# davidlougheed/strkit

Measured on AMD Instinct MI355X. Metric: reads/sec realigned, higher is better.
Workload: dtype int32; 1 GPU; cfg2 shape (1000 loci x 30 HiFi reads, motif 3-6 bp, flank 70), 10000 loci x 30 reads per step and GPU, 8 distinct resident batches in rotation; exact scores (banded first pass with exactness certificate, exact fall-back); distinct_batches=8, parallelism=loci-sharded x1, calls_in_flight=2

## Files before the change

### strkit_amd/csrc/strk_dp_band.h

```cpp
#pragma once

namespace strk {

struct BandLayout {
    int wd, pad, maxdb, maxcol, off_sel, off_cp, cp_bytes, ct_bytes, cp_tail, off_ct, off_b0, group_bytes, sel_len;
    static constexpr int OFF_COMB = 0, OFF_MISC = OFF_COMB + kTableMax * 4, OFF_LMAX = OFF_MISC + 16;
    static constexpr int kBandHiPad = kBandRowSlack + 32;
    __host__ __device__ constexpr BandLayout(int c)
        : wd(128 << c), pad((128 << c) + (8 << c) + 8), maxdb(band_max_db(c)), maxcol(band_max_col(c)),
          off_sel(OFF_LMAX + (band_class_lmax(c) ? kTableMax * 4 : 0)),
          off_cp(off_sel + ((band_max_db(c) + 2 * ((128 << c) + (8 << c) + 8) + kBandHiPad + 15) & ~15)),
          cp_bytes(band_class_fly(c) ? 512 : ((band_max_db(c) + kBandRowSlack + 2 * (8 << c) + 4 + 15) & ~15)),
          ct_bytes((kBandMaxFlank + 2 * (8 << c) + 4 + 15) & ~15),
          cp_tail(c == 0 ? cp_bytes - ct_bytes : cp_bytes),
          off_ct(off_cp + cp_tail),
          off_b0(off_ct + ct_bytes),
          group_bytes(off_b0 + ((band_max_col(c) * 2 + 15) & ~15)),
          sel_len((band_max_db(c) + 2 * ((128 << c) + (8 << c) + 8) + kBandHiPad) & ~3) {}
};
static_assert(band_class_layout(4) == 0 && band_class_layout(7) == 3 && band_class_wd(5) <= band_class_wd(1) && band_class_G(6) == band_class_G(2),
              "a 12-diagonal class uses the LDS layout of the 16-diagonal class with its lane count: pads sized for the wider band cover it");
__host__ __device__ constexpr int band_wave_lds(int c) { return (64 / (8 << c)) * BandLayout(c).group_bytes; }
__host__ __device__ constexpr int max_band_wave_lds(int c) {
    return c < 0 ? 0 : (band_wave_lds(c) > max_band_wave_lds(c - 1) ? band_wave_lds(c) : max_band_wave_lds(c - 1));
}
constexpr int kBandWaveLds = max_band_wave_lds(3);
constexpr int kBandNeg16 = -20000;
constexpr int kBandTblClass0 = 18;
constexpr int kBandSelFront = 5, kBandSelBack = 6;
constexpr int kBandTblBytes = 256;
__host__ __device__ constexpr int band_class_symbol(int c) {
    return c == 0 ? 0 : (c == 1 ? 1 : (c == 2 ? 3 : (c == 3 ? 2 : (c == 4 ? 15 : (c == 7 ? 14 : -1)))));
}
constexpr unsigned kBandLetterLo = 0x47544341u, kBandLetterHi = 0x4E000058u;
typedef const __attribute__((address_space(3))) uint8_t* lds_cu8;

struct BandCtx {
    int lig;
    bool first, last;
    int notFirst, notLast;
    const uint8_t* tbl;
    const uint8_t* selb;
    int pad, maxidx, ndb;
    const uint8_t* flL;
    const uint8_t* motifL;
    int nfl, m;
    int flyP;
};

__device__ __forceinline__ int wave_min_over_groups(int v) {
    int m = __builtin_amdgcn_readlane(v, 0);
#pragma unroll
    for (int l = 8; l < 64; l += 8) m = min(m, __builtin_amdgcn_readlane(v, l));
    return m;
}
template <int G>
__device__ __forceinline__ int from_left0(int v, int notFirst) {
    const int x = __builtin_amdgcn_update_dpp(0, v, G <= 16 ? kDppRowShr1 : kDppWaveShr1, 0xf, 0xf, true);
    return (G == 16 || G == 64) ? x : (x & notFirst);
}
template <int G>
__device__ __forceinline__ int from_right0(int v, int notLast) {
    const int x = __builtin_amdgcn_update_dpp(0, v, G <= 16 ? kDppRowShl1 : kDppWaveShl1, 0xf, 0xf, true);
    return (G == 16 || G == 64) ? x : (x & notLast);
}

template <int G, int D, bool BWD, bool FLY, bool LMAX>
__device__ __forceinline__ void band_pass(const BandCtx& x, const uint8_t* rowsym, int nrows, int dlo_, bool topFree,
                                          bool leftFree, int nEff, int fork0, int m, int cmin, int ncol, int* comb,
                                          short* b0col, int* lmaxA) {
    static_assert(D % 4 == 0 && D >= 8 && D <= 16, "a lane keeps 8, 12 or 16 diagonals");
    constexpr int g = kGap, NQ = D / 4;
    const int ncols = x.ndb;
    const int d0 = dlo_ + x.lig * D;
    auto g0 = [&](int j) -> int { return topFree ? g * min(max(j, 0), ncols) : 0; };
    auto col_addr = [&](int j) -> int {
        return BWD ? x.pad + ncols - j : x.pad + j - 1;
    };
    int Ha[D], Hb[D];
    int Hsave[BWD ? D : 1];
    unsigned sel[NQ];
#pragma unroll
    for (int k = 0; k < (BWD ? D : 1); ++k) Hsave[k] = 0;
#pragma unroll
    for (int k = 0; k < D; ++k) Ha[k] = g0(-x.lig + d0 + k);
    const int jb0 = 1 - x.lig + d0;
    {
#pragma unroll
        for (int q = 0; q < NQ; ++q) {
            unsigned v = 0;
#pragma unroll
            for (int b = 0; b < 4; ++b) v |= (unsigned)x.selb[col_addr(jb0 + 4 * q + b)] << (8 * b);
            sel[q] = v;
        }
    }
    const int T = (wave_max_over_groups(nrows > 0 ? nrows + G - 1 : 0) + 1) & ~1;
    const int dhi_ = dlo_ + D * G - 1;
    int houtL = Ha[D - 1];
    int forkT = (!BWD && nEff > 0) ? fork0 - 1 + x.lig : 0x7fffffff;
    if (BWD && nrows > 0) forkT = nrows - 1 + x.lig;
    int forkIdx = 0;
    int lastmax = kNegInf;
    lds_cu8 psym = FLY ? (lds_cu8)(x.flL + 256 - x.nfl - x.lig) : (lds_cu8)(rowsym + (G - 1) - x.lig);
    lds_cu8 const flyEnd = (lds_cu8)x.motifL + x.flyP;
    lds_cu8 const tbl = (lds_cu8)x.tbl;
    auto row_word = [&](unsigned sym8) -> uint2 {
        const unsigned long long v = *reinterpret_cast<const __attribute__((address_space(3))) unsigned long long*>(tbl + sym8);
        return make_uint2((unsigned)v, (unsigned)(v >> 32));
    };
    uint2 wordE, wordO;
    wordE = row_word(psym[0]);
    wordO = row_word(psym[1]);
    lds_cu8 pnb = (lds_cu8)(x.selb + col_addr(jb0 + D)) - (BWD ? 1 : 0);
#define STRK_BAND_STEP(SRC, DST, TT, ODD, EDGE, FORK)                                              \
    {                                                                                              \
        if (FORK) { STRK_BAND_FORK(SRC, (TT) - 1) }                                                \
        const uint2 word = (ODD) ? wordO : wordE;                                                  \
        unsigned sym2 = (unsigned)psym[2 + (ODD)];                         \
        unsigned nb = pnb[BWD ? 1 - (ODD) : (ODD)];                                                \
        int leftEdge, keepU = 0;                                                                   \
        if (EDGE) {                                                                                \
              \
            const int keepL = ((TT) + dlo_ <= 0 && leftFree) ? g * ((TT) + 1) : 0;                  \
            leftEdge = from_left<G>(keepL, houtL, x.first);                                        \
              \
            const int rl = (TT) - G + 2;                                                           \
            keepU = rl <= 1 ? g0(rl + dhi_) : 0;                                                   \
        } else {                                                                                   \
            leftEdge = from_left0<G>(houtL, x.notFirst);                                           \
        }                                                                                          \
        unsigned wq[NQ];                                                                           \
        _Pragma("unroll") for (int q = 0; q < NQ; ++q) wq[q] = __builtin_amdgcn_perm(word.y, word.x, sel[q]); \
        DST[0] = max(max(SRC[1], leftEdge), SRC[0] + (int)(wq[0] & 0xffu));                        \
        const int upEdge = (EDGE) ? from_right<G>(keepU, DST[0], x.last) : from_right0<G>(DST[0], x.notLast); \
        _Pragma("unroll") for (int k = 1; k < D - 1; ++k)                                          \
            DST[k] = max(max(SRC[k + 1], DST[k - 1]), SRC[k] + (int)((wq[k / 4] >> (8 * (k % 4))) & 0xffu)); \
        DST[D - 1] = max(max(upEdge, DST[D - 2]), SRC[D - 1] + (int)(wq[NQ - 1] >> 24));           \
        houtL = DST[D - 1];                                                                        \
                          \
        asm volatile("" : "+v"(nb), "+v"(sym2));                                                   \
        if (LMAX && !BWD) {                                                                        \
            lastmax = max(lastmax + g, houtL);       \
                                                \
            if ((EDGE) && (TT) == G - 2) lastmax = kNegInf;                                        \
        }                                                                                          \
        _Pragma("unroll") for (int q = 0; q + 1 < NQ; ++q) sel[q] = __builtin_amdgcn_alignbyte(sel[q + 1], sel[q], 1); \
        sel[NQ - 1] = __builtin_amdgcn_alignbyte(nb, sel[NQ - 1], 1);                              \
        if (ODD) wordO = row_word(sym2); else wordE = row_word(sym2);                              \
    }
#define STRK_BAND_FORK(V, TT)                                                                      \
                                                                     \
    if ((!BWD || __builtin_amdgcn_ballot_w64((TT) == forkT) != 0) && (TT) == forkT) {              \
        const int jb = jb0 + (TT);                        \
        if (BWD) {                                                                                 \
                           \
            _Pragma("unroll") for (int k = 0; k < D; ++k)                                          \
                asm volatile("v_mov_b32 %0, %1" : "+v"(Hsave[k]) : "v"(V[k]));                         \
            forkT = 0x7fffffff;                                                                    \
        } else {                                                                                   \
            const short* bc = b0col + (jb - cmin);                                                 \
            int acc = kNegInf;                                                                     \
            _Pragma("unroll") for (int k = 0; k < D; k += 2)                                       \
                acc = max(max(acc, V[k] + (int)bc[k]), V[k + 1] + (int)bc[k + 1]);                 \
            atomicMax(&comb[forkIdx], acc);                                                        \
            if (LMAX && x.last) lmaxA[forkIdx] = lastmax - g * ((TT) + 1 - x.lig);    \
            ++forkIdx;                                                                             \
            forkT = forkIdx < nEff ? forkT + m : 0x7fffffff;                                       \
        }                                                                                          \
    }
    const bool hasL = nrows > 0 && leftFree && dlo_ <= 0;
    const int tTop = (G - 1) & ~1;
    const int tL0 = wave_min_over_groups(hasL ? -dlo_ : 0x3fffffff) & ~1;
    const int tL1 = wave_max_over_groups(hasL ? -dlo_ : -1);
    const int tF = min(T, wave_min_over_groups(BWD ? (nrows > 0 ? nrows - 1 : 0x3fffffff) : (nEff > 0 ? fork0 - 1 : 0x3fffffff)) & ~1);
    auto advance = [&]() {
        psym += 2;
        if (FLY) {
            int past = (int)(flyEnd - psym - 1) >> 31;
            asm volatile("" : "+v"(past));
            psym -= x.flyP & past;
        }
        asm volatile("" : "+v"(psym));
        pnb += BWD ? -2 : 2;
        asm volatile("" : "+v"(pnb));
    };
    int t = 0;
    while (t < T) {
        int ts = T;
        if (tTop >= t) ts = min(ts, tTop);
        if (tL1 >= t) ts = min(ts, max(tL0, t));
        for (const int tn = min(ts, tF); t < tn; t += 2) {
            STRK_BAND_STEP(Ha, Hb, t, 0, false, false)
            STRK_BAND_STEP(Hb, Ha, t + 1, 1, false, false)
            advance();
        }
        for (; t < ts; t += 2) {
            STRK_BAND_STEP(Ha, Hb, t, 0, false, true)
            STRK_BAND_STEP(Hb, Ha, t + 1, 1, false, true)
            advance();
        }
        for (; t < T && (t == tTop || (t >= tL0 && t <= tL1)); t += 2) {
            STRK_BAND_STEP(Ha, Hb, t, 0, true, true)
            STRK_BAND_STEP(Hb, Ha, t + 1, 1, true, true)
            advance();
        }
    }
    STRK_BAND_FORK(Ha, T - 1)
    if (BWD && nrows > 0) {
        const int jb = jb0 + nrows - 1 + x.lig;
#pragma unroll
        for (int k = 0; k < D; ++k) {
            const int jp = jb + k, idx = ncols - jp - cmin;
            if (jp >= 0 && jp <= ncols && idx >= 0 && idx < ncol) b0col[idx] = (short)Hsave[k];
        }
    }
#undef STRK_BAND_STEP
#undef STRK_BAND_FORK
}

template <int BC, class NA, class NB, class NC>
__device__ __forceinline__ void band_wave(const KArgs& a, bool act, int4 q0, int4 q1, int4 q2, uint8_t* Lw, const uint8_t* s_enc,
                                          const uint8_t* s_tbl, NA& nextA, NB& nextB, NC& nextC) {
    constexpr int g = kGap, G = band_class_G(BC), D = band_class_D(BC);
    constexpr bool FLY = band_class_fly(BC);
    constexpr bool LMAX = band_class_lmax(BC);
    constexpr BandLayout lay(band_class_layout(BC));
    const int lane = threadIdx.x & 63;
    int lig_ = lane & (G - 1);
    asm volatile("" : "+v"(lig_));
    const int lig = lig_;
    const int grp = lane / G;
    const bool first = lig == 0, last = lig == G - 1;
    uint8_t* const Lg = Lw + grp * lay.group_bytes;
    int* const comb = reinterpret_cast<int*>(Lg + BandLayout::OFF_COMB);
    int* const misc = reinterpret_cast<int*>(Lg + BandLayout::OFF_MISC);
    int* const lmaxA = reinterpret_cast<int*>(Lg + BandLayout::OFF_LMAX);
    uint8_t* const selb = Lg + lay.off_sel;
    uint8_t* const cp = Lg + lay.off_cp;
    uint8_t* const ct = Lg + lay.off_ct;
    short* const b0col = reinterpret_cast<short*>(Lg + lay.off_b0);
    uint8_t* const motifL = FLY ? cp + 256 : Lg + lay.off_b0;
    constexpr bool TAIL = lay.cp_tail < lay.cp_bytes;
    constexpr int kRowTail = lay.cp_tail - (G - 1);
    static_assert(2 * kBandMaxFlank + kGap * (kBandMaxFlank + band_max_db(1)) < 32767 + kBandNeg16, "b0col: 16-bit columns, kBandNeg16 as -inf");

    int r = 0, nfl = 1, ntr = 0, nfr = 1, m = 1, lo = 0, n = 0;
    long long soff = 0;
    const uint8_t* motif = a.motifs;
    if (act) {
        r = q0.x; nfl = q0.z; ntr = q0.w;
        nfr = q1.x; m = q1.y; lo = q1.z; n = q1.w;
        soff = (long long)(((unsigned long long)(unsigned)q2.y << 32) | (unsigned)q2.x);
        motif += q2.z;
    }
    const int ndb = nfl + ntr + nfr;
    const BandGeo geo = band_geometry_of_class(BC, nfl, ntr, m, lo, max(n, 1), a.band_tune);
    const int rowsP = act ? nfl + (lo + n - 1) * m : 0;
    const int rowsT = act ? nfr : 0;
    const bool dbBeg = a.end_flags & 1, dbEnd = a.end_flags & 2, cBeg = a.end_flags & 4, cEnd = a.end_flags & 8;

    if (first) { misc[0] = 0; misc[1] = act ? q2.z : 0; }
    wave_lds_sync();
    {
        constexpr unsigned kFront = 0x01010101u * kBandSelFront, kBack = 0x01010101u * kBandSelBack;
        constexpr int ND = lay.sel_len / 4, PD = lay.pad / 4;
        constexpr int kBehind = (lay.wd + kBandRowSlack + G + 28 + 3) / 4;
        static_assert(lay.pad % 4 == 0, "the window starts on a dword of the selector array");
        unsigned other = 0;
        const uint8_t* seq = a.seqs + soff;
        unsigned* const selw = reinterpret_cast<unsigned*>(selb);
        const int nd = act ? (ndb + 3) >> 2 : 0;
        for (int d = lig; d < PD; d += G) selw[d] = kFront;
        for (int d = PD + nd + lig; d < min(ND, PD + nd + kBehind); d += G) selw[d] = kBack;
        for (int d0 = lig; d0 < nd; d0 += 8 * G) {
            unsigned w[8];
#pragma unroll
            for (int u = 0; u < 8; ++u) {
                const int d = d0 + u * G;
                unsigned v = 0;
                if (4 * d + 3 < ndb) {
                    __builtin_memcpy(&v, seq + 4 * d, 4);
                } else {
#pragma unroll
                    for (int b = 0; b < 3; ++b)
                        if (4 * d + b < ndb) v |= (unsigned)seq[4 * d + b] << (8 * b);
                }
                w[u] = v;
            }
#pragma unroll
            for (int u = 0; u < 8; ++u) {
                const int d = d0 + u * G;
                unsigned out = (w[u] >> 1) & 0x07070707u;
                unsigned bad = (w[u] & 0xDFDFDFDFu) ^ __builtin_amdgcn_perm(kBandLetterHi, kBandLetterLo, out);
                if (4 * d + 3 >= ndb) {
                    const unsigned vm = 4 * d >= ndb ? 0u : (0xffffffffu >> (8 * (4 * d + 4 - ndb)));
                    out = (out & vm) | (kBack & ~vm);
                    bad &= vm;
                }
                other |= bad;
                if (d < nd) selw[PD + d] = out;
            }
        }
        nextA();
        if (other) misc[0] = 1;
        for (int k = lig; k < m; k += G) motifL[k] = act ? s_enc[motif[k]] : (uint8_t)kNullSym;
    }
    wave_lds_sync();
    const bool fallback = act && misc[0] != 0;
    for (int e = lig; e < kTableMax; e += G) { comb[e] = kNegInf; if (LMAX) lmaxA[e] = kNegInf; }
    {
        if (FLY) {
            for (int k = lig; k < 256; k += G) {
                const int row = k - (256 - nfl);
                cp[k] = (uint8_t)(8 * (row >= 0 ? kBandTblClass0 + selb[lay.pad + row] : kNullSym));
            }
            wave_lds_sync();
            for (int k = lig; k < m; k += G) motifL[k] = (uint8_t)(8 * motifL[k]);
            wave_lds_sync();
            for (int k = m + lig; k < 256; k += G) motifL[k] = motifL[k % m];
        } else {
            const int lenP = wave_max_over_groups(rowsP) + 2 * (G - 1) + 4;
            for (int idx = lig; idx < G - 1; idx += G) cp[idx] = (uint8_t)(8 * kNullSym);
            uint8_t* const cpr = cp + (G - 1);
            for (int row = lig; row < min(min(nfl, rowsP), kRowTail); row += G) cpr[row] = (uint8_t)(8 * (kBandTblClass0 + selb[lay.pad + row]));
            {
                const int gstep = G % m;
                int ph = lig % m;
                for (int row = nfl + lig; row < min(rowsP, kRowTail); row += G) {
                    cpr[row] = (uint8_t)(8 * motifL[ph]);
                    ph += gstep;
                    if (ph >= m) ph -= m;
                }
            }
            for (int row = rowsP + lig; row < min(lenP - (G - 1), kRowTail); row += G) cpr[row] = (uint8_t)(8 * kNullSym);
        }
        const int lenT = wave_max_over_groups(rowsT) + 2 * (G - 1) + 4;
        for (int idx = lig; idx < lenT; idx += G) {
            const int row = idx - (G - 1);
            int sym = kNullSym;
            if (row >= 0 && row < rowsT) sym = kBandTblClass0 + selb[lay.pad + ndb - 1 - row];
            ct[idx] = (uint8_t)(8 * sym);
        }
    }
    wave_lds_sync();
    {
        constexpr unsigned kNeg2 = ((unsigned)(unsigned short)(short)kBandNeg16) * 0x00010001u;
        const int nc2 = min(lay.maxcol, wave_max_over_groups(act ? geo.ncol : 0) + 1) >> 1;
        unsigned* const b2 = reinterpret_cast<unsigned*>(b0col);
        for (int k = lig; k <= nc2; k += G) if (2 * k < lay.maxcol) b2[k] = kNeg2;
    }
    wave_lds_sync();
    nextB();

    if (FLY) {
        const int rmax = wave_max_over_groups(rowsP);
        if (rmax >= 11264) __builtin_amdgcn_s_setprio(3);
        else if (rmax >= 8192) __builtin_amdgcn_s_setprio(2);
        else if (rmax >= 5120) __builtin_amdgcn_s_setprio(1);
    }
    BandCtx x;
    x.lig = lig; x.first = first; x.last = last; x.notFirst = first ? 0 : -1; x.notLast = last ? 0 : -1; x.selb = selb;
    asm volatile("" : "+v"(x.notFirst), "+v"(x.notLast));
    x.pad = lay.pad; x.maxidx = lay.sel_len - 1; x.ndb = ndb;
    x.flL = cp; x.motifL = motifL; x.nfl = nfl; x.m = m;
    x.flyP = FLY ? ((256 - 4) / m) * m : 0;
    const bool run = act && !fallback && geo.ok;
    const int nEff = run ? n : 0;
    x.tbl = s_tbl + kBandTblBytes;
    band_pass<G, D, true, false, false>(x, ct, run ? rowsT : 0, geo.bdlo, dbEnd, cEnd, 0, 0, 1, geo.cmin, geo.ncol, comb, b0col, lmaxA);
    wave_lds_sync();
    nextC();
    if (TAIL) {
        const int lenP = wave_max_over_groups(rowsP) + 2 * (G - 1) + 4;
        uint8_t* const cpr = cp + (G - 1);
        const uint8_t* const mo = a.motifs + misc[1];
        int mm = m, row0 = kRowTail + lig;
        asm volatile("" : "+v"(mm), "+v"(row0));
        for (int row = row0; row < lenP - (G - 1); row += G) {
            int sym = kNullSym;
            if (row < min(nfl, rowsP)) sym = kBandTblClass0 + selb[lay.pad + row];
            else if (row < rowsP) sym = s_enc[mo[(row - nfl) % mm]];
            cpr[row] = (uint8_t)(8 * sym);
        }
        wave_lds_sync();
    }
    x.tbl = s_tbl;
    band_pass<G, D, false, FLY, LMAX>(x, cp, run ? rowsP : 0, geo.dlo, dbBeg, cBeg, nEff, nfl + lo * m, m, geo.cmin, geo.ncol, comb, b0col, lmaxA);
    wave_lds_sync();
    if (FLY) __builtin_amdgcn_s_setprio(0);
    if (run) {
        for (int k = lig; k < n; k += G) {
            const int R = nfl + (lo + k) * m;
            int sc = max(comb[k], -(1 << 28)) - g * (R + nfr + ndb);
            if (LMAX && cEnd) sc = max(sc, max(lmaxA[k], -(1 << 28)) - g * ndb);
            a.table[(long long)r * a.table_stride + k] = sc;
            a.ub[(long long)r * a.table_stride + k] = band_ub(geo, nfl, ntr, nfr, m, lo + k, a.end_flags);
        }
    }
    if (act && first && !run) {
        band_read_to_exact(a, r, nfl, ntr, nfr, m, lo, n);
        a.exact[r] = 1;
    }
    wave_lds_sync();
}

template <int SET>
__device__ __forceinline__ void band_kernel_body(const KArgs& a) {
    constexpr int C0 = SET ? 3 : 1, C1 = SET ? 7 : 5, C2 = SET ? 2 : 0, C3 = SET ? 6 : 4;
    const int n0_ = min(a.counters[kCntClass0 + kBandClass0 + C0], a.list_stride);
    const int n1_ = min(a.counters[kCntClass0 + kBandClass0 + C1], a.list_stride);
    const int n2_ = min(a.counters[kCntClass0 + kBandClass0 + C2], a.list_stride);
    const int n3_ = min(a.counters[kCntClass0 + kBandClass0 + C3], a.list_stride);
    if (n0_ + n1_ + n2_ + n3_ <= 0) return;
    constexpr int kTblBytes = 2 * kBandTblBytes;
    __shared__ __attribute__((aligned(16))) uint8_t lds[kTblBytes + 4 * kBandWaveLds + kLdsSlack];
    __shared__ uint8_t s_enc[256];
    static_assert(2 * (sizeof(lds) + 256) + 4608 <= 160 * 1024, "band kernels: two blocks per CU with room for k_plan's LDS");
    uint8_t* const s_tbl = lds;
    {
        s_enc[threadIdx.x] = c_enc[threadIdx.x];
        if (threadIdx.x < kTblBytes / 8) {
            const int pass = threadIdx.x / (kBandTblBytes / 8), t = threadIdx.x % (kBandTblBytes / 8);
            const bool topFree = a.end_flags & (pass ? 2 : 1), leftFree = a.end_flags & (pass ? 8 : 4);
            const int e = t < kBandTblClass0 ? t : (t < kBandTblClass0 + 8 ? band_class_symbol(t - kBandTblClass0) : -1);
            unsigned long long word = 0;
            for (int k = 0; k < 8; ++k) {
                const int cs = band_class_symbol(k);
                unsigned b = 0;
                if (t == kNullSym) {
                    b = (cs >= 0 && topFree) ? kGap : 0;
                } else if (e >= 0 && e < kNSym) {
                    if (cs >= 0) b = (unsigned)(c_mat[e][cs] + kWBias) & 0xffu;
                    else b = (leftFree && k == (pass ? kBandSelBack : kBandSelFront)) ? kGap : 0;
                }
                word |= (unsigned long long)b << (8 * k);
            }
            reinterpret_cast<unsigned long long*>(s_tbl)[threadIdx.x] = word;
        }
    }
    __syncthreads();
    uint8_t* const Lw = lds + kTblBytes + (threadIdx.x >> 6) * kBandWaveLds;
    constexpr int G01 = band_class_G(C0), G23 = band_class_G(C2);
    constexpr int per01 = 64 / G01, per23 = 64 / G23;
    const int ch0 = (n0_ + per01 - 1) / per01, ch1 = (n1_ + per01 - 1) / per01, ch2 = (n2_ + per23 - 1) / per23, ch3 = (n3_ + per23 - 1) / per23;
    const int e0 = ch0, e1 = e0 + ch1, e2 = e1 + ch2, e3 = e2 + ch3;
    const int lane = threadIdx.x & 63;
    auto pop = [&]() {
        int c = 0;
        if (lane == 0) c = atomicAdd(&a.counters[kCntNextBand + SET], 1);
        return __builtin_amdgcn_readfirstlane(c);
    };
    auto fetch = [&](int c, bool& act, int4& q0, int4& q1, int4& q2) -> int {
        int cls = C0, it = 0, cnt = 0, G_ = G01;
        if (c < e0) { cls = C0; it = c * per01 + lane / G01; cnt = n0_; }
        else if (c < e1) { cls = C1; it = (c - e0) * per01 + lane / G01; cnt = n1_; }
        else if (c < e2) { cls = C2; it = (c - e1) * per23 + lane / G23; cnt = n2_; G_ = G23; }
        else if (c < e3) { cls = C3; it = (c - e2) * per23 + lane / G23; cnt = n3_; G_ = G23; }
        act = it < cnt;
        if (act) {
            const int4* rec = (SET ? a.band_recs_w : a.band_recs) + ((size_t)cls * a.list_stride + it) * 3;
            q0 = rec[0]; q1 = rec[1]; q2 = rec[2];
        }
        return G_;
    };
    auto touch = [&](bool act_, long long so, int ndb_, int G_) -> unsigned {
        unsigned sink = 0;
        if (act_) {
            const uint8_t* pp = a.seqs + so + min((lane & (G_ - 1)) * 64, max(ndb_ - 1, 0));
            asm volatile("global_load_ubyte %0, %1, off" : "=v"(sink) : "v"(pp) : "memory");
        }
        return sink;
    };
    int c = pop();
    bool act = false;
    int4 q0 = make_int4(0, 0, 0, 0), q1 = q0, q2 = q0;
    (void)fetch(c, act, q0, q1, q2);
    while (c < e3) {
        __builtin_amdgcn_wave_barrier();
        int cn_raw = 0, cn = 0, g_n = 8, ndb_n = 0;
        long long so_n = 0;
        bool act_n = false;
        unsigned sink = 0;
        auto nextA = [&]() { if (lane == 0) cn_raw = atomicAdd(&a.counters[kCntNextBand + SET], 1); };
        auto nextB = [&]() {
            int4 n0 = make_int4(0, 0, 0, 0), n1 = n0, n2 = n0;
            cn = __builtin_amdgcn_readfirstlane(cn_raw);
            g_n = fetch(cn, act_n, n0, n1, n2);
            so_n = (long long)(((unsigned long long)(unsigned)n2.y << 32) | (unsigned)n2.x);
            ndb_n = n0.z + n0.w + n1.x;
        };
        auto nextC = [&]() { sink = touch(act_n, so_n, ndb_n, g_n); };
        if (c < e0) band_wave<C0>(a, act, q0, q1, q2, Lw, s_enc, s_tbl, nextA, nextB, nextC);
        else if (c < e1) band_wave<C1>(a, act, q0, q1, q2, Lw, s_enc, s_tbl, nextA, nextB, nextC);
        else if (c < e2) band_wave<C2>(a, act, q0, q1, q2, Lw, s_enc, s_tbl, nextA, nextB, nextC);
        else band_wave<C3>(a, act, q0, q1, q2, Lw, s_enc, s_tbl, nextA, nextB, nextC);
        c = cn;
        (void)fetch(c, act, q0, q1, q2);
        asm volatile("s_waitcnt vmcnt(0)" : : "v"(sink) : "memory");
    }
}
__global__ void __launch_bounds__(256) __attribute__((amdgpu_waves_per_eu(2, 2))) k_dp_band(KArgs a) { band_kernel_body<0>(a); }
__global__ void __launch_bounds__(256) __attribute__((amdgpu_waves_per_eu(2, 2))) k_dp_band_wide(KArgs a) { band_kernel_body<1>(a); }

}
```

### strkit_amd/csrc/strk_kernels.h

```cpp
#pragma once
#include <hip/hip_runtime.h>
#include <stdint.h>

#include "strk_scoring.h"
#include "strk_search.h"
#include "strk_plan_order.h"

namespace strk {

constexpr int kTableMax = 32;
static_assert(kTableMax < 64, "k_plan keeps a band item's table length in six bits");
constexpr int kNegInf = -(1 << 29);
constexpr int kFastFlankMax = 127;
constexpr int kMotifMax = 256;
constexpr int kRowSlack = 160;

constexpr int kNumClasses = 17;
__host__ __device__ constexpr int class_G(int c) { return c < 7 ? 8 : (c < 9 ? 16 : (c < 13 ? 32 : 64)); }
__host__ __device__ constexpr int class_CL(int c) {
    return c < 7 ? 16 + 4 * c : (c < 9 ? 24 + 4 * (c - 7) : (c < 13 ? 16 + 4 * (c - 9) : 16 + 4 * (c - 13)));
}
__host__ __device__ constexpr int class_cap(int c) { return class_G(c) * class_CL(c); }
constexpr int kLongClass = kNumClasses;
constexpr int kGenericClass = kNumClasses + 1;
constexpr int kBandClass0 = kNumClasses + 2;
constexpr int kNumLists = kNumClasses + 2 + kNumBandClasses;
constexpr int kLongTile = 64 * 28;
constexpr int kLongMaxTiles = 64;
constexpr int kLongFlankMax = 255;

__constant__ int8_t c_mat[kNSym][kNSym];
__constant__ uint8_t c_enc[256];

struct KArgs {
    const uint8_t* seqs;
    const int64_t* seq_off;
    const int32_t* nfl;
    const int32_t* ntr;
    const int32_t* nfr;
    const int32_t* est_cn;
    const int32_t* read_off;
    const uint8_t* motifs;
    const int32_t* motif_off;
    int32_t n_reads, n_loci;
    int32_t* read_locus;
    int32_t* win_lo;
    int32_t* win_n;
    int64_t* tab_off;
    int32_t* table;
    int32_t* ub;
    int32_t* cls_list;
    int4* band_recs;
    const int32_t* long_sorted;
    int4* band_recs_w;
    int32_t* wide_hist;
    int32_t* counters;
    unsigned long long* cells;
    int32_t* scratch;
    long long scratch_cap;
    unsigned long long* scratch_used;
    long long long_slot;
    int32_t long_waves;
    int4* spec;
    unsigned long long* rhash;
    int32_t* rep;
    int32_t list_stride;
    int32_t end_flags;
    int32_t window;
    int32_t window_b[5];
    int32_t table_stride;
    int32_t max_iters, lsr, step, tie_last;
    int32_t narrow;
    int32_t band_mode;
    int32_t band_limit;
    BandTune band_tune;
    uint8_t* exact;
    int32_t ref_mode;
};

enum Counter {
    kCntClass0 = 0,
    kCntMiss = kNumLists,
    kCntError = kNumLists + 1,
    kCntNextChunk = kNumLists + 2,
    kCntDup = kNumLists + 3,
    kCntNextLong = kNumLists + 4,
    kCntNextBand = kNumLists + 5,
    kCntBandFallback = kNumLists + 7,
    kCntMissB = kNumLists + 8,
    kCntLociB = kNumLists + 8 + 5,
    kCntTotal = kNumLists + 8 + 10,
    kCntLongNeed = 56
};
static_assert(kCntTotal <= 48 && kCntLongNeed < 64, "counters: 64 ints in front of the 64-bit counters; kCntLongNeed sits in the spare slots");
constexpr int kWinBuckets = 5;
__host__ __device__ constexpr int win_bucket(int m) { return m <= 2 ? 0 : (m <= 4 ? 1 : (m <= 6 ? 2 : (m <= 10 ? 3 : 4))); }
constexpr int kNumWideLists = 4;
__host__ __device__ constexpr int wide_slot(int band_cls) { return (band_cls & 1) | ((band_cls >> 2) << 1); }
__host__ __device__ constexpr int wide_slot_class(int slot) { return 2 + (slot & 1) + ((slot >> 1) << 2); }
__host__ __device__ constexpr int wide_bucket(int rows) { return rows >= (255 << 6) ? 255 : (rows < 0 ? 0 : rows >> 6); }
constexpr int kCellBand = 6, kCellWide = 7, kCellExact = 8, kCellLong = 9;
__host__ __device__ constexpr int cell_slot_of_list(int c) {
    return c >= kBandClass0 ? (band_class_wide_kernel(c - kBandClass0) ? kCellWide : kCellBand)
                            : (c == kLongClass ? kCellLong : (c == kGenericClass ? -1 : kCellExact));
}
constexpr int kErrBadInput = 1;
constexpr int kErrScratch = 2;
constexpr int kErrEmpty = 4;
constexpr int kErrList = 8;
constexpr int kErrLongSlot = 16;

__device__ inline int classify(int nfl, int ntr, int nfr, int m, int lo, int n, int force_generic, int ref_mode) {
    const long long ndb = (long long)nfl + ntr + nfr;
    const long long rows = (long long)nfl + (long long)(lo + n - 1) * m;
    if (force_generic || nfl < 1 || (nfr < 1 && !ref_mode) || n > kTableMax || m > kMotifMax) return kGenericClass;
    for (int c = ref_mode ? kNumClasses - 1 : 0; c < kNumClasses; ++c) {
        const int cap = class_cap(c);
        if (ndb + 1 <= cap && rows <= cap + kRowSlack && (nfr <= kFastFlankMax || ref_mode)) return c;
    }
    if (!ref_mode && nfl <= kLongFlankMax && nfr <= kLongFlankMax && ndb + 1 <= (long long)kLongTile * kLongMaxTiles &&
        rows <= (1 << 20))
        return kLongClass;
    return kGenericClass;
}

__device__ inline void band_read_to_exact(const KArgs& a, int r, int nfl, int ntr, int nfr, int m, int lo, int n) {
    const int c = classify(nfl, ntr, nfr, m, lo, n, 0, 0);
    const int idx = atomicAdd(&a.counters[kCntClass0 + c], 1);
    if (idx < a.list_stride) {
        int32_t* gl = a.cls_list + (size_t)c * a.list_stride * 2;
        gl[2 * idx] = r;
        gl[2 * idx + 1] = 0;
    } else {
        atomicOr(&a.counters[kCntError], kErrList);
    }
    atomicAdd(&a.counters[kCntBandFallback], 1);
    if (c != kGenericClass) {
        const unsigned long long cc = (unsigned long long)(nfl + ntr + nfr) * ((unsigned long long)nfl + (unsigned long long)(lo + n - 1) * m + nfr);
        atomicAdd(a.cells, cc);
        atomicAdd(a.cells + cell_slot_of_list(c), cc);
    }
}

__device__ __forceinline__ unsigned long long hash_mix(unsigned long long h, unsigned long long v) {
    h ^= v;
    h *= 0x9E3779B97F4A7C15ull;
    return h ^ (h >> 29);
}

__global__ void __launch_bounds__(256) k_hash(KArgs a) {
    const int gid = blockIdx.x * blockDim.x + threadIdx.x;
    const int r = gid >> 3, sl = gid & 7;
    const bool act = r < a.n_reads;
    unsigned long long h = 0xCBF29CE484222325ull + (unsigned long long)sl;
    if (act) {
        const uint8_t* p = a.seqs + a.seq_off[r];
        const int len = (int)(a.seq_off[r + 1] - a.seq_off[r]);
        const int nw = (len + 7) >> 3;
        for (int w = sl; w < nw; w += 8) {
            unsigned long long v = 0;
            const int i = w << 3;
            if (i + 8 <= len) __builtin_memcpy(&v, p + i, 8);
            else for (int k = 0; i + k < len; ++k) v |= (unsigned long long)p[i + k] << (8 * k);
            h = hash_mix(h, v + 0x9E3779B97F4A7C15ull * (unsigned long long)(w + 1));
        }
    }
#pragma unroll
    for (int o = 1; o < 8; o <<= 1) {
        const unsigned long long other = (unsigned long long)__shfl_down((long long)h, o, 8);
        h = hash_mix(h, other);
    }
    if (act && sl == 0) {
        h = hash_mix(h, ((unsigned long long)(unsigned)a.nfl[r] << 32) | (unsigned)a.ntr[r]);
        h = hash_mix(h, ((unsigned long long)(unsigned)a.nfr[r] << 32) | (unsigned)a.est_cn[r]);
        a.rhash[r] = h;
    }
}

__device__ inline bool same_read(const KArgs& a, int r, int q) {
    if (a.nfl[r] != a.nfl[q] || a.ntr[r] != a.ntr[q] || a.nfr[r] != a.nfr[q] || a.est_cn[r] != a.est_cn[q]) return false;
    const uint8_t* x = a.seqs + a.seq_off[r];
    const uint8_t* y = a.seqs + a.seq_off[q];
    const int len = a.nfl[r] + a.ntr[r] + a.nfr[r];
    int i = 0;
    for (; i + 32 <= len; i += 32) {
        unsigned long long u0, u1, u2, u3, v0, v1, v2, v3;
        __builtin_memcpy(&u0, x + i, 8); __builtin_memcpy(&u1, x + i + 8, 8); __builtin_memcpy(&u2, x + i + 16, 8); __builtin_memcpy(&u3, x + i + 24, 8);
        __builtin_memcpy(&v0, y + i, 8); __builtin_memcpy(&v1, y + i + 8, 8); __builtin_memcpy(&v2, y + i + 16, 8); __builtin_memcpy(&v3, y + i + 24, 8);
        if ((u0 ^ v0) | (u1 ^ v1) | (u2 ^ v2) | (u3 ^ v3)) return false;
    }
    for (; i + 8 <= len; i += 8) {
        unsigned long long u, v;
        __builtin_memcpy(&u, x + i, 8);
        __builtin_memcpy(&v, y + i, 8);
        if (u != v) return false;
    }
    for (; i < len; ++i)
        if (x[i] != y[i]) return false;
    return true;
}

__device__ inline int first_identical(const KArgs& a, int r, int q0) {
    const unsigned long long h = a.rhash[r];
    int q = q0;
    for (;;) {
        int cand = r;
        for (; q < r && cand == r; q += 4) {
            const unsigned long long h0 = a.rhash[q], h1 = a.rhash[min(q + 1, r)], h2 = a.rhash[min(q + 2, r)], h3 = a.rhash[min(q + 3, r)];
            const int k = h0 == h ? 0 : (h1 == h ? 1 : (h2 == h ? 2 : (h3 == h ? 3 : 4)));
            if (k < 4 && q + k < r) cand = q + k;
        }
        if (cand == r) return r;
        if (same_read(a, r, cand)) return cand;
        q = cand + 1;
    }
}

__global__ void __launch_bounds__(kPlanThreads) k_plan(KArgs a, int mode, const int32_t* items, int n_items, int force_generic, int rpt) {
    __shared__ int s_cnt[kNumLists];
    __shared__ int s_base[kNumLists];
    __shared__ unsigned long long s_cells, s_bytes_band, s_bytes_exact, s_bytes_wide, s_bytes_long, s_cells_k[4];
    __shared__ int s_bin[kPlanBins];
    __shared__ int s_wsum[kPlanWaves];
    __shared__ int s_below[kNumBandClasses];
    __shared__ int s_lb[kWinBuckets];
    const int tid = threadIdx.x, lane = tid & 63, wave = tid >> 6;
    if (tid < kWinBuckets) s_lb[tid] = 0;
    if (tid < kNumLists) s_cnt[tid] = 0;
    if (tid == 0) { s_cells = 0; s_bytes_band = 0; s_bytes_exact = 0; s_bytes_wide = 0; s_bytes_long = 0; }
    if (tid < 4) s_cells_k[tid] = 0;
    for (int b = tid; b < kPlanBins; b += kPlanThreads) s_bin[b] = 0;
    __syncthreads();
    int p_key[kPlanReadsPerThread];
#pragma unroll
    for (int k = 0; k < kPlanReadsPerThread; ++k) p_key[k] = -1;
#pragma unroll 1
    for (int j = 0; j < rpt; ++j) {
        const int gid = blockIdx.x * (kPlanThreads * rpt) + j * kPlanThreads + tid;
        int r = 0, l = 0, nfl = 0, ntr = 0, nfr = 0, m = 1, lo = 0, n = 0;
        if (gid < n_items) {
            r = items ? items[gid] : gid;
            int lo_l = 0, hi_l = a.n_loci;
            while (hi_l - lo_l > 1) {
                const int mid = (lo_l + hi_l) >> 1;
                if (a.read_off[mid] <= r) lo_l = mid; else hi_l = mid;
            }
            l = lo_l;
            a.read_locus[r] = l;
            m = a.motif_off[l + 1] - a.motif_off[l];
            if (mode == 0 && r == a.read_off[l] && m >= 1) atomicAdd(&s_lb[win_bucket(m)], 1);
            nfl = a.nfl[r]; ntr = a.ntr[r]; nfr = a.nfr[r];
            if (m < 1 || nfl < 0 || ntr < 0 || nfr < 0) {
                atomicOr(&a.counters[kCntError], kErrBadInput);
                a.win_n[r] = 0;
                n = 0;
            } else if (mode == 0) {
                const long long est = a.est_cn[r];
                const long long w = min((long long)a.window_b[win_bucket(m)] + min(max(est, 0ll) >> 7, 7ll), (long long)(a.table_stride - 1) / 2);
                long long w_lo = est - w, w_hi = est + w;
                if (w_lo < 0) w_lo = 0;
                if (w_hi < w_lo) w_hi = w_lo;
                if (w_hi - w_lo + 1 > a.table_stride) w_hi = w_lo + a.table_stride - 1;
                lo = (int)w_lo;
                n = (int)(w_hi - w_lo + 1);
                const int rep = a.rhash ? first_identical(a, r, a.read_off[l]) : r;
                a.rep[r] = rep;
                if (a.spec) a.spec[r] = make_int4(0, 0, 0, kSpecMiss);
                a.win_lo[r] = lo;
                a.win_n[r] = n;
                a.tab_off[r] = (int64_t)rep * a.table_stride;
                if (rep != r) {
                    n = 0;
                    atomicAdd(&a.counters[kCntDup], 1);
                }
            } else {
                lo = a.win_lo[r];
                n = a.win_n[r];
            }
        }
        unsigned long long cells = 0;
        const unsigned long long ndb = (unsigned long long)nfl + ntr + nfr;
        int band_list = -1;
        if (a.band_mode && mode == 0 && n > 0 && n <= kTableMax && !force_generic && r < a.band_limit) {
            const BandGeo geo = band_geometry(nfl, ntr, nfr, m, lo, n, a.band_tune);
            if (geo.ok) band_list = kBandClass0 + geo.cls;
        }
        if (a.exact && gid < n_items && n > 0) a.exact[r] = band_list < 0;
        int first_c = -1;
        for (int k0 = 0; k0 < n; k0 += kTableMax) {
            const int nn = min(kTableMax, n - k0);
            const int c = band_list >= 0 ? band_list : classify(nfl, ntr, nfr, m, lo + k0, nn, force_generic, a.ref_mode);
            if (k0 == 0) first_c = c;
            atomicAdd(&s_cnt[c], 1);
            unsigned long long cc = 0;
            if (c == kGenericClass) {
                for (int k = 0; k < nn; ++k) cc += ndb * ((unsigned long long)nfl + (unsigned long long)(lo + k0 + k) * m + nfr);
            } else if (band_list >= 0) {
                cc = (unsigned long long)band_class_wd(band_list - kBandClass0) * ((unsigned long long)nfl + (unsigned long long)(lo + k0 + nn - 1) * m + nfr);
            } else {
                cc = ndb * ((unsigned long long)nfl + (unsigned long long)(lo + k0 + nn - 1) * m + nfr);
            }
            cells += cc;
            if (cc && cell_slot_of_list(c) >= 0) atomicAdd(&s_cells_k[cell_slot_of_list(c) - kCellBand], cc);
        }
        if (cells) {
            atomicAdd(&s_cells, cells);
            atomicAdd(band_list >= 0 ? &s_bytes_band : &s_bytes_exact, ndb + 16);
            if (band_list >= 0 && band_class_wide_kernel(band_list - kBandClass0)) atomicAdd(&s_bytes_wide, ndb + 16);
            if (first_c == kLongClass) atomicAdd(&s_bytes_long, ndb + 16);
        }
        int key = -(n + 1);
        if (band_list >= 0) {
            const int bin = plan_bin(band_list - kBandClass0, nfl + (lo + n - 1) * m);
            atomicAdd(&s_bin[bin], 1);
            key = ((band_list - kBandClass0) << 18) | (n << 12) | bin;
        }
#pragma unroll
        for (int k = 0; k < kPlanReadsPerThread; ++k) p_key[k] = k == j ? key : p_key[k];
    }
    __syncthreads();
    if (tid < kNumLists) {
        const int c = tid;
        s_base[c] = s_cnt[c] ? atomicAdd(&a.counters[kCntClass0 + c], s_cnt[c]) : 0;
    }
    int bin_cnt[kPlanBinsPerThread], own = 0;
#pragma unroll
    for (int k = 0; k < kPlanBinsPerThread; ++k) {
        const int b = tid * kPlanBinsPerThread + k;
        bin_cnt[k] = b < kPlanBins ? s_bin[b] : 0;
        own += bin_cnt[k];
    }
    int incl = own;
#pragma unroll
    for (int o = 1; o < 64; o <<= 1) {
        const int v = __shfl_up(incl, o);
        if (lane >= o) incl += v;
    }
    if (lane == 63) s_wsum[wave] = incl;
    __syncthreads();
    if (tid < kNumBandClasses) {
        int below = 0;
        for (int k = 0; k < tid; ++k) below += s_cnt[kBandClass0 + k];
        s_below[tid] = below;
    }
    {
        int pre = incl - own;
        for (int w = 0; w < wave; ++w) pre += s_wsum[w];
#pragma unroll
        for (int k = 0; k < kPlanBinsPerThread; ++k) {
            const int b = tid * kPlanBinsPerThread + k;
            if (b < kPlanBins) s_bin[b] = pre;
            pre += bin_cnt[k];
        }
    }
    __syncthreads();
    if (tid < kNumLists) s_cnt[tid] = 0;
    if (tid < kWinBuckets && s_lb[tid]) atomicAdd(&a.counters[kCntLociB + tid], s_lb[tid]);
    if (tid == 0 && s_cells) {
        atomicAdd(a.cells, s_cells);
        if (s_bytes_band) atomicAdd(a.cells + 2, s_bytes_band);
        if (s_bytes_exact) atomicAdd(a.cells + 3, s_bytes_exact);
        if (s_bytes_wide) atomicAdd(a.cells + 4, s_bytes_wide);
        if (s_bytes_long) atomicAdd(a.cells + 5, s_bytes_long);
        for (int k = 0; k < 4; ++k)
            if (s_cells_k[k]) atomicAdd(a.cells + kCellBand + k, s_cells_k[k]);
    }
#pragma unroll
    for (int j = 0; j < kPlanReadsPerThread; ++j) {
        if (j >= rpt) break;
        const int bin = p_key[j] >= 0 ? (p_key[j] & 0xfff) : -1;
        int rank = 0, group = 0, leader = 0;
        unsigned long long todo = __ballot(bin >= 0);
        while (todo) {
            const int first = __ffsll((long long)todo) - 1;
            const int b = __shfl(bin, first);
            const unsigned long long same = __ballot(bin == b);
            if (bin == b) {
                rank = __popcll(same & ((1ull << lane) - 1));
                group = __popcll(same);
                leader = first;
            }
            todo &= ~same;
        }
        int base = 0;
        for (int w = 0; w < kPlanWaves; ++w) {
            if (w == wave && bin >= 0 && lane == leader) {
                base = s_bin[bin];
                s_bin[bin] = base + group;
            }
            __syncthreads();
        }
        base = __shfl(base, leader);
        if (bin >= 0) p_key[j] = (p_key[j] & ~0xfff) | (base + rank);
    }
#pragma unroll
    for (int j = 0; j < kPlanReadsPerThread; ++j) {
        const int band_cls = p_key[j] >= 0 ? (p_key[j] >> 18) : -1;
        const int n = p_key[j] >= 0 ? ((p_key[j] >> 12) & 63) : -(p_key[j] + 1);
        if (n <= 0) continue;
        const int gid = blockIdx.x * (kPlanThreads * rpt) + j * kPlanThreads + tid;
        const int r = items ? items[gid] : gid;
        const int l = a.read_locus[r], lo = a.win_lo[r];
        const int nfl = a.nfl[r], ntr = a.ntr[r], nfr = a.nfr[r], m = a.motif_off[l + 1] - a.motif_off[l];
        const int band_list = band_cls >= 0 ? kBandClass0 + band_cls : -1;
        for (int k0 = 0; k0 < n; k0 += kTableMax) {
            const int nn = min(kTableMax, n - k0);
            const int c = band_list >= 0 ? band_list : classify(nfl, ntr, nfr, m, lo + k0, nn, force_generic, a.ref_mode);
            const int idx = s_base[c] + (band_list >= 0 ? (p_key[j] & 0xfff) - s_below[band_cls] : atomicAdd(&s_cnt[c], 1));
            if (idx < a.list_stride) {
                a.cls_list[(size_t)c * a.list_stride * 2 + 2 * idx] = r;
                a.cls_list[(size_t)c * a.list_stride * 2 + 2 * idx + 1] = band_list >= 0 ? l : k0;
                if (band_list >= 0) {
                    int4* rec = a.band_recs + ((size_t)band_cls * a.list_stride + idx) * 3;
                    const long long so = a.seq_off[r];
                    rec[0] = make_int4(r, l, nfl, ntr);
                    rec[1] = make_int4(nfr, m, lo, n);
                    rec[2] = make_int4((int)(so & 0xffffffffll), (int)(so >> 32), a.motif_off[l], a.est_cn[r]);
                }
            } else {
                atomicOr(&a.counters[kCntError], kErrList);
            }
        }
    }
}

__global__ void __launch_bounds__(64) k_scalar_plan(KArgs a, int n_counter_ints) {
    for (int i = threadIdx.x; i < n_counter_ints; i += 64) a.counters[i] = 0;
    __syncthreads();
    if (threadIdx.x != 0) return;
    const int nfl = a.nfl[0], ntr = a.ntr[0], nfr = a.nfr[0], m = a.motif_off[1] - a.motif_off[0];
    a.read_locus[0] = 0;
    a.tab_off[0] = 0;
    a.spec[0] = make_int4(0, 0, 0, kSpecMiss);
    a.win_lo[0] = 0;
    a.win_n[0] = 0;
    if (m < 1 || nfl < 0 || ntr < 0 || nfr < 0) { a.counters[kCntError] = kErrBadInput; return; }
    const long long est = a.est_cn[0];
    const long long w = min((long long)a.window + min(max(est, 0ll) >> 7, 7ll), (long long)(a.table_stride - 1) / 2);
    long long w_lo = est - w, w_hi = est + w;
    if (w_lo < 0) w_lo = 0;
    if (w_hi < w_lo) w_hi = w_lo;
    if (w_hi - w_lo + 1 > a.table_stride) w_hi = w_lo + a.table_stride - 1;
    const int lo = (int)w_lo, n = (int)(w_hi - w_lo + 1);
    a.win_lo[0] = lo;
    a.win_n[0] = n;
    int c = classify(nfl, ntr, nfr, m, lo, n, 0, 0);
    if (c < kNumClasses) {
        const long long ndb = (long long)nfl + ntr + nfr, rows = (long long)nfl + (long long)(lo + n - 1) * m;
        long long best = -1;
        for (int k = c; k < kNumClasses; ++k) {
            const int cap = class_cap(k);
            if (ndb + 1 > cap || rows > cap + kRowSlack) continue;
            const long long cost = (rows + nfr + 2 * class_G(k)) * (9 * class_CL(k) / 4 + 12);
            if (best < 0 || cost < best) { best = cost; c = k; }
        }
        a.cls_list[(size_t)c * a.list_stride * 2] = 0;
        a.cls_list[(size_t)c * a.list_stride * 2 + 1] = 0;
        a.counters[kCntClass0 + c] = 1;
    }
}

constexpr int kSortWideBlocks = 16;
__device__ __forceinline__ int wide_rec_bucket(const int4* recs, int idx) {
    const int4 q0 = recs[(size_t)idx * 3], q1 = recs[(size_t)idx * 3 + 1];
    return 255 - wide_bucket(q0.z + (q1.z + q1.w - 1) * q1.y);
}
__global__ void __launch_bounds__(256) k_sort_wide_hist(KArgs a) {
    __shared__ int s_hist[256];
    const int s = blockIdx.y, cls = wide_slot_class(s);
    const int count = min(a.counters[kCntClass0 + kBandClass0 + cls], a.list_stride);
    if (count <= 0) return;
    const int4* recs = a.band_recs + (size_t)cls * a.list_stride * 3;
    s_hist[threadIdx.x] = 0;
    __syncthreads();
    for (int i = blockIdx.x * 256 + threadIdx.x; i < count; i += kSortWideBlocks * 256) atomicAdd(&s_hist[wide_rec_bucket(recs, i)], 1);
    __syncthreads();
    if (s_hist[threadIdx.x]) atomicAdd(&a.wide_hist[s * 256 + threadIdx.x], s_hist[threadIdx.x]);
}
__global__ void __launch_bounds__(256) k_sort_wide(KArgs a, int4* out) {
    __shared__ int s_cnt[256], s_base[256], s_wave[4];
    const int s = blockIdx.y, cls = wide_slot_class(s);
    const int count = min(a.counters[kCntClass0 + kBandClass0 + cls], a.list_stride);
    if (count <= 0) return;
    const int4* recs = a.band_recs + (size_t)cls * a.list_stride * 3;
    s_cnt[threadIdx.x] = 0;
    __syncthreads();
    for (int i = blockIdx.x * 256 + threadIdx.x; i < count; i += kSortWideBlocks * 256) atomicAdd(&s_cnt[wide_rec_bucket(recs, i)], 1);
    __syncthreads();
    {
        const int lane = threadIdx.x & 63, w = threadIdx.x >> 6;
        const int v = a.wide_hist[s * 256 + threadIdx.x];
        int incl = v;
        for (int o = 1; o < 64; o <<= 1) {
            const int u = __shfl_up(incl, o, 64);
            if (lane >= o) incl += u;
        }
        if (lane == 63) s_wave[w] = incl;
        __syncthreads();
        int base = incl - v;
        for (int k = 0; k < w; ++k) base += s_wave[k];
        const int mine = s_cnt[threadIdx.x];
        s_base[threadIdx.x] = mine ? base + atomicAdd(&a.wide_hist[(kNumWideLists + s) * 256 + threadIdx.x], mine) : 0;
        s_cnt[threadIdx.x] = 0;
    }
    __syncthreads();
    for (int i = blockIdx.x * 256 + threadIdx.x; i < count; i += kSortWideBlocks * 256) {
        const int4 q0 = recs[(size_t)i * 3], q1 = recs[(size_t)i * 3 + 1], q2 = recs[(size_t)i * 3 + 2];
        const int b = 255 - wide_bucket(q0.z + (q1.z + q1.w - 1) * q1.y);
        const int pos = s_base[b] + atomicAdd(&s_cnt[b], 1);
        int4* o = out + ((size_t)cls * a.list_stride + pos) * 3;
        o[0] = q0; o[1] = q1; o[2] = q2;
    }
}

__global__ void __launch_bounds__(1024) k_sort_long(KArgs a, int32_t* out) {
    __shared__ int s_hist[1024], s_start[1024];
    const int count = min(a.counters[kCntClass0 + kLongClass], a.list_stride);
    if (count <= 0) return;
    const int32_t* list = a.cls_list + (size_t)kLongClass * a.list_stride * 2;
    s_hist[threadIdx.x] = 0;
    __syncthreads();
    auto bucket_of = [&](int r, int k0) {
        const int l = a.read_locus[r];
        const int m = a.motif_off[l + 1] - a.motif_off[l];
        const long long ndb = (long long)a.nfl[r] + a.ntr[r] + a.nfr[r];
        const long long rows = (long long)a.nfl[r] + (long long)(a.win_lo[r] + k0 + min(kTableMax, a.win_n[r] - k0) - 1) * m;
        const long long cost = ((ndb + kLongTile) / kLongTile) * (rows + 64);
        return 1023 - (int)min(1023ll, cost >> 9);
    };
    for (int i = threadIdx.x; i < count; i += 1024) atomicAdd(&s_hist[bucket_of(list[2 * i], list[2 * i + 1])], 1);
    __syncthreads();
    {
        __shared__ int s_wave[16];
        const int lane = threadIdx.x & 63, w = threadIdx.x >> 6;
        const int v = s_hist[threadIdx.x];
        int incl = v;
        for (int o = 1; o < 64; o <<= 1) {
            const int u = __shfl_up(incl, o, 64);
            if (lane >= o) incl += u;
        }
        if (lane == 63) s_wave[w] = incl;
        __syncthreads();
        int base = 0;
        for (int k = 0; k < w; ++k) base += s_wave[k];
        s_start[threadIdx.x] = base + incl - v;
        s_hist[threadIdx.x] = 0;
    }
    __syncthreads();
    for (int i = threadIdx.x; i < count; i += 1024) {
        const int r = list[2 * i], k0 = list[2 * i + 1];
        const int b = bucket_of(r, k0);
        const int pos = s_start[b] + atomicAdd(&s_hist[b], 1);
        out[2 * pos] = r;
        out[2 * pos + 1] = k0;
    }
}

}

#include "strk_dp_exact.h"
#include "strk_dp_band.h"
#include "strk_dp_long.h"
#include "strk_replay.h"
```

Measured before the change: 312.5 million reads/s.

## Stage band row symbols by dwords and cheapen the read-dedup hash

New measurement: 319.0 million reads/s (median of 6 runs). No clear change (+2.1%).

```diff
diff --git a/strkit_amd/csrc/strk_band_stage.h b/strkit_amd/csrc/strk_band_stage.h
--- /dev/null
+++ b/strkit_amd/csrc/strk_band_stage.h
@@ -0,0 +1,68 @@
+#pragma once
+
+#include <cstdint>
+
+#include "strk_search.h"
+
+namespace strk {
+
+constexpr int32_t kBandStageClass0 = 18;
+constexpr uint32_t kBandStageNull4 = 0x01010101u * (8u * 17u);
+STRK_HD uint32_t band_low_bytes(int32_t k) {
+    const int32_t c = k < 0 ? 0 : (k > 4 ? 4 : k);
+    return (uint32_t)~(~0ull << (8 * c));
+}
+STRK_HD uint32_t band_flank_rows4(uint32_t sel4) { return (sel4 << 3) + 0x01010101u * (8u * kBandStageClass0); }
+STRK_HD uint32_t band_bswap4(uint32_t v) { return (v >> 24) | ((v >> 8) & 0xff00u) | ((v << 8) & 0xff0000u) | (v << 24); }
+STRK_HD uint32_t band_back_rows4(uint32_t sel4, int32_t r0, int32_t rowsT) {
+    const uint32_t valid = band_low_bytes(rowsT - r0) & ~band_low_bytes(-r0);
+    return (band_flank_rows4(band_bswap4(sel4)) & valid) | (kBandStageNull4 & ~valid);
+}
+STRK_HD uint32_t band_load4(const uint8_t* p) { uint32_t v; __builtin_memcpy(&v, p, 4); return v; }
+STRK_HD void band_store4(uint8_t* p, uint32_t v) { __builtin_memcpy(p, &v, 4); }
+
+template <int G>
+STRK_HD void band_stage_back_rows(uint8_t* ct, const uint8_t* win, int32_t ndb, int32_t rowsT, int32_t lenT, int32_t lig) {
+    for (int32_t j = lig; 4 * j < lenT; j += G) {
+        const int32_t r0 = 4 * j - (G - 1);
+        band_store4(ct + 4 * j, band_back_rows4(band_load4(win + ndb - 4 - r0), r0, rowsT));
+    }
+}
+
+struct BandRowEnds { int32_t e1, e2, e3; };
+STRK_HD BandRowEnds band_row_ends(int32_t G, int32_t nfl, int32_t rowsP, int32_t lenP, int32_t lim) {
+    const int32_t nflE = nfl < rowsP ? nfl : rowsP, rows = rowsP > nflE ? rowsP : nflE;
+    BandRowEnds e;
+    e.e1 = G - 1 + nflE < lim ? G - 1 + nflE : lim;
+    e.e2 = G - 1 + rows < lim ? G - 1 + rows : lim;
+    e.e3 = lenP < lim ? lenP : lim;
+    return e;
+}
+template <int G>
+STRK_HD void band_stage_flank_rows(uint8_t* cp, const uint8_t* win, BandRowEnds e, int32_t lig) {
+    uint32_t nf = band_low_bytes(G - 1 - 4 * lig);
+    for (int32_t j = lig; 4 * j < e.e1; j += G) {
+        band_store4(cp + 4 * j, (band_flank_rows4(band_load4(win + 4 * j - (G - 1))) & ~nf) | (kBandStageNull4 & nf));
+        nf = 0;
+    }
+}
+template <int G>
+STRK_HD void band_stage_motif_rows(uint8_t* cp, const uint8_t* motif3, int32_t m, BandRowEnds e, int32_t lig) {
+    const int32_t h1 = (-e.e1) & 3;
+    if (lig < h1 && e.e1 + lig < e.e2) cp[e.e1 + lig] = (uint8_t)(8 * motif3[lig]);
+    const uint32_t um = (uint32_t)m, pstep = (4u * G) % um;
+    uint32_t ph = (uint32_t)(h1 + 4 * lig) % um;
+    for (int32_t c = e.e1 + h1 + 4 * lig; c < e.e2; c += 4 * G) {
+        band_store4(cp + c, band_load4(motif3 + ph) << 3);
+        ph += pstep;
+        if (ph >= um) ph -= um;
+    }
+}
+template <int G>
+STRK_HD void band_stage_null_rows(uint8_t* cp, BandRowEnds e, int32_t lig) {
+    const int32_t h2 = (-e.e2) & 3;
+    if (lig < h2 && e.e2 + lig < e.e3) cp[e.e2 + lig] = (uint8_t)(8 * 17);
+    for (int32_t c = e.e2 + h2 + 4 * lig; c < e.e3; c += 4 * G) band_store4(cp + c, kBandStageNull4);
+}
+
+}
diff --git a/strkit_amd/csrc/strk_dp_band.h b/strkit_amd/csrc/strk_dp_band.h
--- a/strkit_amd/csrc/strk_dp_band.h
+++ b/strkit_amd/csrc/strk_dp_band.h
@@ -1,4 +1,6 @@
 #pragma once
+
+#include "strk_band_stage.h"
 
 namespace strk {
 
@@ -27,6 +29,7 @@
 constexpr int kBandWaveLds = max_band_wave_lds(3);
 constexpr int kBandNeg16 = -20000;
 constexpr int kBandTblClass0 = 18;
+static_assert(kBandStageClass0 == kBandTblClass0 && kBandStageNull4 == 0x01010101u * (8u * kNullSym), "strk_band_stage.h <-> the row-word tables");
 constexpr int kBandSelFront = 5, kBandSelBack = 6;
 constexpr int kBandTblBytes = 256;
 __host__ __device__ constexpr int band_class_symbol(int c) {
@@ -280,7 +283,7 @@
                 unsigned v = 0;
                 if (4 * d + 3 < ndb) {
                     __builtin_memcpy(&v, seq + 4 * d, 4);
-                } else {
+                } else if (d < nd) {
 #pragma unroll
                     for (int b = 0; b < 3; ++b)
                         if (4 * d + b < ndb) v |= (unsigned)seq[4 * d + b] << (8 * b);
@@ -290,6 +293,7 @@
 #pragma unroll
             for (int u = 0; u < 8; ++u) {
                 const int d = d0 + u * G;
+                if (d >= nd) continue;
                 unsigned out = (w[u] >> 1) & 0x07070707u;
                 unsigned bad = (w[u] & 0xDFDFDFDFu) ^ __builtin_amdgcn_perm(kBandLetterHi, kBandLetterLo, out);
                 if (4 * d + 3 >= ndb) {
@@ -298,12 +302,21 @@
                     bad &= vm;
                 }
                 other |= bad;
-                if (d < nd) selw[PD + d] = out;
+                selw[PD + d] = out;
             }
         }
         nextA();
         if (other) misc[0] = 1;
-        for (int k = lig; k < m; k += G) motifL[k] = act ? s_enc[motif[k]] : (uint8_t)kNullSym;
+        const int mext = FLY ? m : m + 3;
+        for (int k = lig; k < mext; k += G) {
+            int kk = k;
+            if (!FLY) {
+                kk = kk >= m ? kk - m : kk;
+                kk = kk >= m ? kk - m : kk;
+                kk = kk >= m ? kk - m : kk;
+            }
+            motifL[k] = act ? s_enc[motif[kk]] : (uint8_t)kNullSym;
+        }
     }
     wave_lds_sync();
     const bool fallback = act && misc[0] != 0;
@@ -319,28 +332,18 @@
             wave_lds_sync();
             for (int k = m + lig; k < 256; k += G) motifL[k] = motifL[k % m];
         } else {
+            static_assert(FLY || (((band_max_db(band_class_layout(BC)) + kBandRowSlack + 2 * (G - 1) + 4 + 3) & ~3) <= lay.cp_bytes && lay.cp_tail % 4 == 0),
+                          "cp by dwords: the last dword lies inside cp, and the part staged here ends on a dword");
             const int lenP = wave_max_over_groups(rowsP) + 2 * (G - 1) + 4;
-            for (int idx = lig; idx < G - 1; idx += G) cp[idx] = (uint8_t)(8 * kNullSym);
-            uint8_t* const cpr = cp + (G - 1);
-            for (int row = lig; row < min(min(nfl, rowsP), kRowTail); row += G) cpr[row] = (uint8_t)(8 * (kBandTblClass0 + selb[lay.pad + row]));
-            {
-                const int gstep = G % m;
-                int ph = lig % m;
-                for (int row = nfl + lig; row < min(rowsP, kRowTail); row += G) {
-                    cpr[row] = (uint8_t)(8 * motifL[ph]);
-                    ph += gstep;
-                    if (ph >= m) ph -= m;
-                }
-            }
-            for (int row = rowsP + lig; row < min(lenP - (G - 1), kRowTail); row += G) cpr[row] = (uint8_t)(8 * kNullSym);
+            const BandRowEnds re = band_row_ends(G, nfl, rowsP, lenP, lay.cp_tail);
+            band_stage_flank_rows<G>(cp, selb + lay.pad, re, lig);
+            band_stage_motif_rows<G>(cp, motifL, m, re, lig);
+            band_stage_null_rows<G>(cp, re, lig);
         }
         const int lenT = wave_max_over_groups(rowsT) + 2 * (G - 1) + 4;
-        for (int idx = lig; idx < lenT; idx += G) {
-            const int row = idx - (G - 1);
-            int sym = kNullSym;
-            if (row >= 0 && row < rowsT) sym = kBandTblClass0 + selb[lay.pad + ndb - 1 - row];
-            ct[idx] = (uint8_t)(8 * sym);
-        }
+        static_assert(lay.pad + 2 - 4 - (kBandMaxFlank + (G - 1) + 3) >= 0 && ((kBandMaxFlank + 2 * (G - 1) + 4 + 3) & ~3) <= lay.ct_bytes,
+                      "ct by dwords: the selector bytes of every staged row lie inside the array, the last dword inside ct");
+        band_stage_back_rows<G>(ct, selb + lay.pad, ndb, rowsT, lenT, lig);
     }
     wave_lds_sync();
     {
diff --git a/strkit_amd/csrc/strk_kernels.h b/strkit_amd/csrc/strk_kernels.h
--- a/strkit_amd/csrc/strk_kernels.h
+++ b/strkit_amd/csrc/strk_kernels.h
@@ -148,11 +148,19 @@
     return h ^ (h >> 29);
 }
 
+struct HashAcc { unsigned x, y; };
+__host__ __device__ __forceinline__ unsigned hash_rotr(unsigned v, int s) { return (v >> s) | (v << (32 - s)); }
+__host__ __device__ __forceinline__ HashAcc hash_word(HashAcc h, unsigned lo, unsigned hi) {
+    h.x = (h.x ^ lo) + h.y;
+    h.y = hash_rotr(h.y ^ hi, 21) + h.x;
+    return h;
+}
+
 __global__ void __launch_bounds__(256) k_hash(KArgs a) {
     const int gid = blockIdx.x * blockDim.x + threadIdx.x;
     const int r = gid >> 3, sl = gid & 7;
     const bool act = r < a.n_reads;
-    unsigned long long h = 0xCBF29CE484222325ull + (unsigned long long)sl;
+    HashAcc h = {0x84222325u + (unsigned)sl, 0xCBF29CE4u};
     if (act) {
         const uint8_t* p = a.seqs + a.seq_off[r];
         const int len = (int)(a.seq_off[r + 1] - a.seq_off[r]);
@@ -160,20 +168,31 @@
         for (int w = sl; w < nw; w += 8) {
             unsigned long long v = 0;
             const int i = w << 3;
-            if (i + 8 <= len) __builtin_memcpy(&v, p + i, 8);
-            else for (int k = 0; i + k < len; ++k) v |= (unsigned long long)p[i + k] << (8 * k);
-            h = hash_mix(h, v + 0x9E3779B97F4A7C15ull * (unsigned long long)(w + 1));
-        }
-    }
-#pragma unroll
-    for (int o = 1; o < 8; o <<= 1) {
-        const unsigned long long other = (unsigned long long)__shfl_down((long long)h, o, 8);
-        h = hash_mix(h, other);
-    }
+            if (i + 8 <= len) {
+                __builtin_memcpy(&v, p + i, 8);
+            } else if (len >= 8) {
+                __builtin_memcpy(&v, p + len - 8, 8);
+                v >>= 8 * (i + 8 - len);
+            } else {
+                for (int k = 0; i + k < len; ++k) v |= (unsigned long long)p[i + k] << (8 * k);
+            }
+            h = hash_word(h, (unsigned)v, (unsigned)(v >> 32));
+        }
+    }
+#define STRK_HASH_FOLD(CTRL)                                                                          \
+    {                                                                                                 \
+        const unsigned ox = (unsigned)__builtin_amdgcn_update_dpp(0, (int)h.x, CTRL, 0xf, 0xf, true);  \
+        const unsigned oy = (unsigned)__builtin_amdgcn_update_dpp(0, (int)h.y, CTRL, 0xf, 0xf, true);  \
+        h = hash_word(h, ox, oy);                                                                     \
+    }
+    STRK_HASH_FOLD(0x101)
+    STRK_HASH_FOLD(0x102)
+    STRK_HASH_FOLD(0x104)
+#undef STRK_HASH_FOLD
     if (act && sl == 0) {
-        h = hash_mix(h, ((unsigned long long)(unsigned)a.nfl[r] << 32) | (unsigned)a.ntr[r]);
-        h = hash_mix(h, ((unsigned long long)(unsigned)a.nfr[r] << 32) | (unsigned)a.est_cn[r]);
-        a.rhash[r] = h;
+        h = hash_word(h, (unsigned)a.nfl[r], (unsigned)a.ntr[r]);
+        h = hash_word(h, (unsigned)a.nfr[r], (unsigned)a.est_cn[r]);
+        a.rhash[r] = hash_mix(((unsigned long long)h.y << 32) | h.x, 0);
     }
 }
 
```
